# frankcholula/sapr

Hardware: AMD Instinct MI355X
Metric: frames/sec MFCC+Viterbi (16kHz, 13-MFCC, 8-state HMM) (higher is better)
Workload: dtype f32 (MFCC) + f64 (trellis); 1 GPU; configs[1]+[2]: 16 kHz 1 s utterances -> 13 MFCC (25 ms/10 ms, n_fft 512, 40 mels) -> Viterbi vs 11 word models x 8 emitting states (decoder.py API), features materialised in HBM; utterances_per_gpu=100000, frames_per_utterance=101, word_models=11, states=10, parallelism=utterance-shard x1, decoder=pruned

## Files before the change

### sapr_amd/csrc/mfcc.hip

```cpp
#include <cmath>
#include <algorithm>
#include <cstdlib>
#include <cstring>
#include <functional>
#include <mutex>
#include <type_traits>
#include <vector>

#include "sapr_common.h"

#pragma clang fp contract(fast)

#ifndef SAPR_ABLATE
#define SAPR_ABLATE 0
#endif

namespace sapr {
namespace {

constexpr int kThreads = 256;
constexpr int kWaves = kThreads / kWave;
constexpr double kPi = 3.14159265358979323846264338327950288;

typedef float f32x4 __attribute__((ext_vector_type(4)));
// ... 1213 lines not shown
    const char *sel = std::getenv("SAPR_MFCC_MEL");
    d.mel_bf16 = (d.ksr && sel && std::strcmp(sel, "bf16") == 0) ? 1 : 0;
  }
  auto lds_total = [&](int ml) {
    const int tp = d.two_pass ? 0 : d.t_pad;
    return R == 16 ? lds_layout<16>(tp, d.lm_stride, d.total_ks, ml, d.n_mels, d.stage_floats).total
                   : lds_layout<32>(tp, d.lm_stride, d.total_ks, ml, d.n_mels, d.stage_floats).total;
  };
  auto pick_mel = [&]() {
    if (d.ksr) return 0;
    return lds_total(1) <= 80 * 1024 || (lds_total(0) > 80 * 1024 && lds_total(1) <= 160 * 1024) ? 1 : 0;
  };
  d.mel_in_lds = pick_mel();
  if (!d.two_pass && lds_total(d.mel_in_lds) > 160 * 1024) {
    d.two_pass = 1;
    d.mel_in_lds = pick_mel();
  }
  if (!d.two_pass && lds_total(d.mel_in_lds) > 80 * 1024) {
    const char *keep = std::getenv("SAPR_MFCC_FUSED");
    MfccDev t = d;
    t.two_pass = 1;
    auto total_of = [&](const MfccDev &x, int ml) {
      return R == 16 ? lds_layout<16>(0, x.lm_stride, x.total_ks, ml, x.n_mels, x.stage_floats).total
                     : lds_layout<32>(0, x.lm_stride, x.total_ks, ml, x.n_mels, x.stage_floats).total;
    };
    const int ml2 = t.ksr ? 0 : ((total_of(t, 1) <= 80 * 1024 || (total_of(t, 0) > 80 * 1024 && total_of(t, 1) <= 160 * 1024)) ? 1 : 0);
    if (!(keep && keep[0] == '1') && total_of(t, ml2) <= 80 * 1024) {
      d.two_pass = 1;
      d.mel_in_lds = ml2;
    }
  }
  pl->lds_bytes = static_cast<size_t>(lds_total(d.mel_in_lds));
  if (pl->lds_bytes > 160 * 1024) {
    (void)hipFree(devbuf);
    const size_t need = pl->lds_bytes;
    delete pl;
    return fail(SAPR_ERR_UNSUPPORTED, "configuration needs %zu bytes of LDS (> 160 KiB)", need);
  }
  if (d.wave_s4) {
    d.two_pass = 1;
    pl->wave_rlo = (d.r_lo >= 1 && d.r_hi <= 15) ? 1 : 0;
    pl->wave_rhi = (d.r_lo >= 1 && d.r_hi <= 15) ? 15 : 16;
    pl->wave_lds = static_cast<size_t>(wave_lds(d.wave_s4, wave_region_floats(d.n_mels, d.deltas)).total);
    pl->lds_bytes = pl->wave_lds;
    hipError_t oe = wave_dispatch(*pl, &pl->wave_blocks_per_cu, nullptr, nullptr, nullptr, 0, 0, 1, nullptr, nullptr,
                                  nullptr, 0, nullptr);
    if (oe != hipSuccess || pl->wave_blocks_per_cu < 1) {
      (void)hipFree(devbuf);
      delete pl;
      return hip_fail(oe, "occupancy query (mfcc_wave_kernel)");
    }
    if (const char *sl = std::getenv("SAPR_MFCC_SLICES")) {
      const int v = std::atoi(sl);
      pl->slices_env = v < 1 ? 0 : (v > kMaxSlices ? kMaxSlices : v);
    }
    {
      int dev = 0, lds_cu = 0;
      if (hipGetDevice(&dev) != hipSuccess ||
          hipDeviceGetAttribute(&lds_cu, hipDeviceAttributeMaxSharedMemoryPerMultiprocessor, dev) != hipSuccess ||
          lds_cu < 64 * 1024)
        lds_cu = 160 * 1024;
      constexpr int kGranule = 320 * 4;
      const int spec = align_up(static_cast<int>(pl->wave_lds), kGranule) * pl->wave_blocks_per_cu;
      const int fin = align_up(static_cast<int>(wave_finish_lds(d.n_mels, d.deltas)), kGranule);
      const int fit = spec < lds_cu ? (lds_cu - spec) / fin : 0;
      pl->finish_beside = fit < 1 ? 1 : (fit > SAPR_FINISH_OCC ? SAPR_FINISH_OCC : fit);
    }
  }
  *plan_out = pl;
  return 0;
}

extern "C" int sapr_mfcc_plan_destroy(void *plan) {
  if (!plan) return 0;
  MfccPlan *pl = static_cast<MfccPlan *>(plan);
  plan_side_destroy(*pl, nullptr);
  if (pl->buffer) (void)hipFree(pl->buffer);
  delete pl;
  return 0;
}

extern "C" int sapr_mfcc_plan_info(const void *plan, int32_t *d_out, int32_t *max_frames,
                                   int64_t *lds_bytes, int32_t *mel_ksteps) {
  SAPR_REQUIRE(plan != nullptr, "plan is NULL");
  const MfccPlan *pl = static_cast<const MfccPlan *>(plan);
  if (d_out) *d_out = pl->dev.d_out;
  if (max_frames) *max_frames = pl->dev.two_pass ? 0 : pl->dev.t_pad;
  if (lds_bytes) *lds_bytes = static_cast<int64_t>(pl->lds_bytes);
  if (mel_ksteps) *mel_ksteps = pl->dev.total_ks;
  return 0;
}

extern "C" int sapr_mfcc_batch_stamped(const void *plan, const float *pcm, const int64_t *sample_offsets,
                                       const int64_t *frame_offsets, int64_t n_utts, float *out,
                                       int32_t grid_blocks, uint64_t *stamps, void *stream) {
  SAPR_REQUIRE(plan && pcm && sample_offsets && frame_offsets && out && stamps, "NULL pointer argument");
  const MfccPlan *pl = static_cast<const MfccPlan *>(plan);
  SAPR_REQUIRE(pl->R == 16 && pl->dev.preemph == 0.f && pl->dev.ksr == kKsr, "stamped build: bench preset only");
  SAPR_REQUIRE(grid_blocks > 0 && grid_blocks <= n_utts, "bad grid");
  if (pl->dev.mel_bf16) {
    if (pl->lds_bytes > 64 * 1024)
      SAPR_HIP_TRY(hipFuncSetAttribute(reinterpret_cast<const void *>(&mfcc_kernel<16, false, false, kKsr, true, false, true>),
                                       hipFuncAttributeMaxDynamicSharedMemorySize, static_cast<int>(pl->lds_bytes)));
    SAPR_LAUNCH((mfcc_kernel<16, false, false, kKsr, true, false, true>), dim3(grid_blocks), dim3(kThreads),
                pl->lds_bytes, as_stream(stream), pcm, sample_offsets, frame_offsets, n_utts, pl->dev, out,
                reinterpret_cast<unsigned long long *>(stamps));
  } else {
    if (pl->lds_bytes > 64 * 1024)
      SAPR_HIP_TRY(hipFuncSetAttribute(reinterpret_cast<const void *>(&mfcc_kernel<16, false, false, kKsr, true>),
                                       hipFuncAttributeMaxDynamicSharedMemorySize, static_cast<int>(pl->lds_bytes)));
    SAPR_LAUNCH((mfcc_kernel<16, false, false, kKsr, true>), dim3(grid_blocks), dim3(kThreads), pl->lds_bytes,
                as_stream(stream), pcm, sample_offsets, frame_offsets, n_utts, pl->dev, out,
                reinterpret_cast<unsigned long long *>(stamps));
  }
  SAPR_HIP_TRY(hipGetLastError());
  return 0;
}

extern "C" int sapr_mfcc_workspace_bytes(const void *plan, int64_t total_frames, int64_t n_utts, size_t *bytes) {
  SAPR_REQUIRE(plan && bytes && total_frames >= 0 && n_utts >= 0, "bad arguments");
  const MfccPlan *pl = static_cast<const MfccPlan *>(plan);
  *bytes = pl->dev.two_pass
               ? (static_cast<size_t>(total_frames) * pl->dev.n_mels + static_cast<size_t>(n_utts)) * sizeof(float) + 256
               : 0;
  return 0;
}

extern "C" int sapr_mfcc_batch(const void *plan, const float *pcm, const int64_t *sample_offsets,
                               const int64_t *frame_offsets, int64_t n_utts, int64_t total_frames, float *out,
                               int32_t grid_blocks, void *workspace, size_t workspace_size, void *stream) {
  SAPR_REQUIRE(plan != nullptr, "plan is NULL");
  SAPR_REQUIRE(n_utts >= 0 && total_frames >= 0, "bad sizes");
  if (n_utts == 0) return 0;
  SAPR_REQUIRE(pcm && sample_offsets && frame_offsets && out, "NULL pointer argument");
  const MfccPlan *pl = static_cast<const MfccPlan *>(plan);
  int dev = 0, cus = 256;
  SAPR_HIP_TRY(hipGetDevice(&dev));
  SAPR_HIP_TRY(hipDeviceGetAttribute(&cus, hipDeviceAttributeMultiprocessorCount, dev));
  int grid = grid_blocks;
  if (grid <= 0) {
    const int per_cu = static_cast<int>((160 * 1024) / pl->lds_bytes);
    const int cap = 3;
    grid = cus * (per_cu < 1 ? 1 : (per_cu > cap ? cap : per_cu));
  }
  if (grid > n_utts) grid = static_cast<int>(n_utts);
  hipStream_t st = as_stream(stream);
  if (!pl->dev.two_pass) {
    if (pl->R == 16)
      SAPR_HIP_TRY((launch<16, false>(*pl, pcm, sample_offsets, frame_offsets, n_utts, out, grid, st, nullptr, nullptr)));
    else
      SAPR_HIP_TRY((launch<32, false>(*pl, pcm, sample_offsets, frame_offsets, n_utts, out, grid, st, nullptr, nullptr)));
    return 0;
  }
  const size_t need = (static_cast<size_t>(total_frames) * pl->dev.n_mels + static_cast<size_t>(n_utts)) * sizeof(float) + 256;
  if (!workspace || workspace_size < need)
    return fail(SAPR_ERR_WORKSPACE, "two-pass MFCC plan needs a %zu-byte workspace (sapr_mfcc_workspace_bytes)", need);
  float *lm = static_cast<float *>(workspace);
  unsigned *gmax = reinterpret_cast<unsigned *>(lm + static_cast<size_t>(total_frames) * pl->dev.n_mels);
  if (pl->dev.wave_s4) {
    const int full_grid = cus * pl->wave_blocks_per_cu;
    const int64_t n_waves_full = static_cast<int64_t>(full_grid) * kWaves;
    const size_t flds = wave_finish_lds(pl->dev.n_mels, pl->dev.deltas);
    const int64_t *fo_end = frame_offsets + n_utts;
    auto finish = [&](hipStream_t s, int64_t u0, int64_t n, int fgrid, int fill) -> hipError_t {
      const int64_t fwaves = static_cast<int64_t>(fgrid) * kWaves;
      int fsplit = 1;
      if (n < fwaves) {
        fsplit = static_cast<int>(std::min<int64_t>(8, fwaves / n));
        const int64_t need_blocks = (n * fsplit + kWaves - 1) / kWaves;
        if (need_blocks < fgrid) fgrid = static_cast<int>(need_blocks);
      }
      SAPR_LAUNCH(mfcc_wave_finish_kernel, dim3(fgrid), dim3(kThreads), flds, s, lm, gmax + u0, frame_offsets + u0, n,
                  pl->dev, out, fsplit, total_frames, fo_end, fill);
      return hipGetLastError();
    };

    int n_slices = 1;
    if (grid_blocks <= 0 && pl->slices_env != 1) {
      if (pl->slices_env > 1) {
        n_slices = pl->slices_env;
      } else {
        n_slices = kDefaultSlices;
        const int64_t fwaves = static_cast<int64_t>(cus) * SAPR_FINISH_OCC * kWaves;
        while (n_slices > 1 && (n_utts / n_slices < fwaves || total_frames / n_slices < 4 * kSliceMinSets * n_waves_full))
          n_slices >>= 1;
      }
      if (n_slices > n_utts) n_slices = static_cast<int>(n_utts);
      if (n_slices > 1) {
        hipStreamCaptureStatus cap = hipStreamCaptureStatusNone;
        if (hipStreamIsCapturing(st, &cap) != hipSuccess || cap != hipStreamCaptureStatusNone) {
          (void)hipGetLastError();
          n_slices = 1;
        }
      }
    }
    if (n_slices > 1) {
      std::lock_guard<std::mutex> lock(pl->side_mu);
      if (!pl->side_tried) {
        pl->side_tried = true;
        int least = 0, greatest = 0;
        hipStream_t s = nullptr;
        bool ok = hipDeviceGetStreamPriorityRange(&least, &greatest) == hipSuccess &&
                  hipStreamCreateWithPriority(&s, hipStreamNonBlocking, least) == hipSuccess;
        for (int k = 0; ok && k < kMaxSlices; ++k) {
          hipEvent_t *e = k < kMaxSlices - 1 ? &pl->ev_spec[k] : &pl->ev_side;
          ok = hipEventCreateWithFlags(e, hipEventDisableTiming) == hipSuccess;
        }
        if (ok) {
          pl->side = s;
        } else {
          (void)hipGetLastError();
          plan_side_destroy(*pl, s);
        }
      }
      if (pl->side) {
        SAPR_HIP_TRY(hipMemsetAsync(gmax, 0, static_cast<size_t>(n_utts) * sizeof(unsigned), st));
        const int beside_grid = cus * pl->finish_beside;
        for (int k = 0; k < n_slices; ++k) {
          const int64_t u0 = n_utts * k / n_slices, n = n_utts * (k + 1) / n_slices - u0;
          SAPR_HIP_TRY(wave_dispatch(*pl, nullptr, pcm, sample_offsets + u0, frame_offsets + u0, n, full_grid, 0, st, lm,
                                     gmax + u0, total_frames, fo_end));
          if (k + 1 < n_slices) {
            SAPR_HIP_TRY(hipEventRecord(pl->ev_spec[k], st));
            SAPR_HIP_TRY(hipStreamWaitEvent(pl->side, pl->ev_spec[k], 0));
            SAPR_HIP_TRY(finish(pl->side, u0, n, beside_grid, 0));
          } else {
            SAPR_HIP_TRY(finish(st, u0, n, cus * SAPR_FINISH_OCC, 1));
          }
        }
        SAPR_HIP_TRY(hipEventRecord(pl->ev_side, pl->side));
        SAPR_HIP_TRY(hipStreamWaitEvent(st, pl->ev_side, 0));
        return 0;
      }
    }
    int wgrid = grid_blocks > 0 ? grid_blocks : full_grid;
    const int64_t n_waves = static_cast<int64_t>(wgrid) * kWaves;
    int64_t span = (total_frames + n_waves - 1) / n_waves;
    span = span < 4 ? 4 : (span + 3) / 4 * 4;
    const int64_t need_blocks = ((total_frames + span - 1) / span + kWaves - 1) / kWaves;
    if (need_blocks < wgrid) wgrid = static_cast<int>(need_blocks < 1 ? 1 : need_blocks);
    SAPR_HIP_TRY(hipMemsetAsync(gmax, 0, static_cast<size_t>(n_utts) * sizeof(unsigned), st));
    SAPR_HIP_TRY(wave_dispatch(*pl, nullptr, pcm, sample_offsets, frame_offsets, n_utts, wgrid, span, st, lm, gmax,
                               total_frames, fo_end));
    SAPR_HIP_TRY(finish(st, 0, n_utts, cus * SAPR_FINISH_OCC, 1));
    return 0;
  } else if (pl->R == 16)
    SAPR_HIP_TRY((launch<16, true>(*pl, pcm, sample_offsets, frame_offsets, n_utts, out, grid, st, lm, gmax)));
  else
    SAPR_HIP_TRY((launch<32, true>(*pl, pcm, sample_offsets, frame_offsets, n_utts, out, grid, st, lm, gmax)));
  int fgrid = cus * 6;
  if (fgrid > n_utts) fgrid = static_cast<int>(n_utts);
  SAPR_LAUNCH(mfcc_finish_kernel, dim3(fgrid), dim3(kThreads), finish_lds_bytes(pl->dev), st, lm, gmax, frame_offsets,
              n_utts, pl->dev, out);
  SAPR_HIP_TRY(hipGetLastError());
  return 0;
}
```

### sapr_amd/csrc/mfcc_wave.h

```cpp
#pragma once

constexpr int kWRowPad = 18;
constexpr int kWGroup = 16 * kWRowPad;
constexpr int kWRegion = 4 * kWGroup;
#include "mfcc_wave_pack.h"

struct WaveLds {
  int win, twab, twu, mela, dtab, scr, total;
};
__host__ __device__ inline int wave_region_floats(int, int) { return kWRegion; }
__host__ __device__ inline WaveLds wave_lds(int s4, int region_floats) {
  WaveLds L;
  int o = 0;
  L.win = o;
  o += 512 * 4;
  L.twab = o;
  o += 256 * 8;
  L.twu = o;
  o += 128 * 8;
  L.mela = o;
  o += s4 * kWave * 16;
  L.dtab = o;
  o += 2 * 81 * 4 + 8;
  L.scr = o;
// ... 161 lines not shown
#pragma unroll
        for (int c4 = 0; c4 < 4; ++c4) {
          const int idx = lane + kWave * c4;
          if (idx < rows * P.n_mfcc) {
            const int tl = static_cast<int>((static_cast<float>(idx) + 0.5f) * inv_nm), c = idx - tl * P.n_mfcc;
            const int t = 16 * e + tl;
            float d1 = 0.f, d2 = 0.f;
            if (t >= 4 && t < T - 4) {
#pragma unroll
              for (int k = 0; k < 9; ++k) {
                const float x = ceps(t - 4 + k, c);
                d1 += dc1[k] * x;
                d2 += dc2[k] * x;
              }
            } else {
              const int row = t < 4 ? 1 + t : 5 + (t - (T - 4)), t0 = t < 4 ? 0 : T - 9;
#pragma unroll
              for (int k = 0; k < 9; ++k) {
                const float x = ceps(t0 + k, c);
                d1 += s_dtab[row * 9 + k] * x;
                d2 += s_dtab[81 + row * 9 + k] * x;
              }
            }
            float *ot = o + tl * P.d_out + c;
            ot[0] = ceps(t, c);
            ot[P.n_mfcc] = d1;
            ot[2 * P.n_mfcc] = d2;
          }
        }
      }
      wave_fence();
    }
  };
  float4 t0[4], t1[4], t2[4];
  if (first < last) fetch(first, t0);
  if (first + 1 < last) fetch(first + 1, t1);
  if (first + 2 < last) fetch(first + 2, t2);
  const int end = last + (deltas ? 1 : 0);
  for (int base = first; base < end; base += 3) {
    tile(base, t0);
    if (base + 1 < end) tile(base + 1, t1);
    if (base + 2 < end) tile(base + 2, t2);
  }
}

#ifndef SAPR_FINISH_OCC
#define SAPR_FINISH_OCC 3
#endif
__global__ __launch_bounds__(kThreads, SAPR_FINISH_OCC) void mfcc_wave_finish_kernel(const float *__restrict__ lm,
                                                                       const unsigned *__restrict__ gmax_enc,
                                                                       const int64_t *__restrict__ frame_offsets,
                                                                       int64_t n_utts, MfccDev P, float *__restrict__ out,
                                                                       int split, int64_t total_cap,
                                                                       const int64_t *__restrict__ batch_end,
                                                                       int fill_on_mismatch) {
  extern __shared__ __attribute__((aligned(16))) unsigned char smem[];
  float *s_dtab = reinterpret_cast<float *>(smem);
  const int per_wave = 16 * (P.n_mels + 4) + (P.deltas ? 3 : 1) * 256;
  const int tid = threadIdx.x;
  const int wave = __builtin_amdgcn_readfirstlane(tid / kWave), lane = tid % kWave;
  for (int i = tid; i < 2 * 81; i += kThreads) s_dtab[i] = P.delta_tab[i];
  for (int i = tid; i < kWaves * per_wave; i += kThreads) s_dtab[168 + i] = 0.f;
  __syncthreads();
  float *s_tile = s_dtab + 168 + wave * per_wave;
  const int n_waves = gridDim.x * kWaves;
  const int wid = blockIdx.x * kWaves + wave;
  if (*batch_end > total_cap) {
    if (!fill_on_mismatch) return;
    const int64_t n = total_cap * P.d_out;
    for (int64_t i = static_cast<int64_t>(blockIdx.x) * kThreads + tid; i < n; i += static_cast<int64_t>(gridDim.x) * kThreads)
      out[i] = __builtin_nanf("");
    return;
  }
  const int n_teams = n_waves / split, part = wid % split;
  if (wid >= n_teams * split) return;
  for (int64_t u = wid / split; u < n_utts; u += n_teams) {
    const int64_t f_beg = frame_offsets[u];
    const int T = static_cast<int>(frame_offsets[u + 1] - f_beg);
    const int n_tiles = (T + 15) >> 4, per = (n_tiles + split - 1) / split;
    const int lo = part * per, hi = lo + per < n_tiles ? lo + per : n_tiles;
    if (lo >= hi) continue;
    wave_finish(lm + f_beg * P.n_mels, T, dec_ordered(gmax_enc[u]) - P.top_db, out + f_beg * P.d_out, P, s_tile,
                s_tile + 16 * (P.n_mels + 4), s_dtab, lane, lo, hi);
  }
}
inline size_t wave_finish_lds(int n_mels, int deltas) {
  return static_cast<size_t>(168 + kWaves * (16 * (n_mels + 4) + (deltas ? 3 : 1) * 256)) * 4;
}

#ifndef SAPR_WAVE_OCC
#define SAPR_WAVE_OCC 4
#endif

template <bool PREEMPH, int RLO, int RHI, int S4>
__global__ __launch_bounds__(kThreads, SAPR_WAVE_OCC) void mfcc_wave_kernel(
    const float *__restrict__ pcm, const int64_t *__restrict__ sample_offsets,
    const int64_t *__restrict__ frame_offsets, int64_t n_utts, MfccDev P, float *__restrict__ lm_out,
    unsigned *__restrict__ gmax_enc, int64_t span, int64_t total_cap, const int64_t *__restrict__ batch_end) {
  constexpr int R = 16, kNc = 256, kBits = 4, NR = RHI - RLO;
  extern __shared__ __attribute__((aligned(16))) unsigned char smem[];
  const int region_floats = wave_region_floats(P.n_mels, P.deltas);
  const WaveLds L = wave_lds(S4, region_floats);
  float *s_win = reinterpret_cast<float *>(smem + L.win);
  float2 *s_twab = reinterpret_cast<float2 *>(smem + L.twab);
  float2 *s_twu = reinterpret_cast<float2 *>(smem + L.twu);
  float4 *s_a = reinterpret_cast<float4 *>(smem + L.mela);
  float *s_dtab = reinterpret_cast<float *>(smem + L.dtab);
  float *s_scr = reinterpret_cast<float *>(smem + L.scr);

  const int tid = threadIdx.x;
  const int wave = __builtin_amdgcn_readfirstlane(tid / kWave);
  const int lane = tid % kWave;

  for (int i = tid; i < 512; i += kThreads) s_win[i] = P.window[i];
  for (int i = tid; i < 256; i += kThreads) s_twab[i] = P.tw_ab[i];
  for (int i = tid; i < 128; i += kThreads) s_twu[i] = P.tw_u[i];
  for (int i = tid; i < S4 * kWave; i += kThreads) s_a[i] = reinterpret_cast<const float4 *>(P.wave_a)[i];
  for (int i = tid; i < 2 * 81; i += kThreads) s_dtab[i] = P.delta_tab[i];
  for (int i = tid; i < kWaves * region_floats; i += kThreads) s_scr[i] = 0.f;
  __syncthreads();

  const int grp = lane >> 4;
  const int l = lane & 15;
  const int sigma = l < 8 ? l : (l == 15 ? 8 : l + 1);
  const bool is0 = l == 0;
  [[maybe_unused]] const bool special = l == 0 || l == 15;
  const unsigned long long special_mask = 0x8001800180018001ull;
  float *region = s_scr + wave * region_floats;
  float *scr = region + grp * kWGroup;
  float *prow = region + grp * kWPRow;
  const int rot = (grp & 1) * 8;
  float *wlo = scr + rot * kWRowPad + l;
  float *whi = scr + (rot ? -8 : 0) * kWRowPad + l;
  const unsigned a_rrow = lds_addr(scr + ((sigma + rot) & 15) * kWRowPad);
  const unsigned a_twu = lds_addr(s_twu + sigma);
  const unsigned a_twab = lds_addr(s_twab + l);
  const unsigned a_win = lds_addr(reinterpret_cast<const float2 *>(s_win) + l);

  const int j4 = lane & 3;
  const int4 bi = reinterpret_cast<const int4 *>(P.wave_blk)[lane >> 2];
  const float4 *bq = reinterpret_cast<const float4 *>(region + j4 * kWPRow + bi.x);
  const float4 *aq = s_a + lane;
  const int mel0 = bi.y;
  const float f1 = bi.z ? 1.f : 0.f, f2 = bi.w ? 1.f : 0.f;

  const int64_t base = frame_offsets[0], total = frame_offsets[n_utts];
  const int64_t wid = static_cast<int64_t>(blockIdx.x) * kWaves + wave;
  if (*batch_end > total_cap) return;
  if (span == 0) {
    const int64_t n_waves = static_cast<int64_t>(gridDim.x) * kWaves;
    span = (total - base + n_waves - 1) / n_waves;
    span = span < 4 ? 4 : (span + 3) / 4 * 4;
  }
  const int64_t run_lo = base + wid * span;
  if (run_lo >= total) return;
  const int64_t run_hi = run_lo + span < total ? run_lo + span : total;
  int64_t u_first = 0;
  {
    int64_t hi = n_utts;
    while (hi - u_first > 1) {
      const int64_t mid = (u_first + hi) >> 1;
      if (frame_offsets[mid] <= run_lo)
        u_first = mid;
      else
        hi = mid;
    }
  }

  for (int64_t u = u_first; u < n_utts; ++u) {
    const int64_t f_beg = frame_offsets[u];
    if (f_beg >= run_hi) break;
    const int T = static_cast<int>(frame_offsets[u + 1] - f_beg);
    const int n_sets = (T + 3) >> 2;
    const int s_lo = f_beg >= run_lo ? 0 : static_cast<int>((run_lo - f_beg + 3) >> 2);
    const int s_hi_raw = static_cast<int>((run_hi - f_beg + 3) >> 2);
    const int s_hi = s_hi_raw < n_sets ? s_hi_raw : n_sets;
    if (s_lo >= s_hi) continue;
    const int64_t s_beg = sample_offsets[u];
    const int n_samp = static_cast<int>(sample_offsets[u + 1] - s_beg);
    const __amdgpu_buffer_rsrc_t rsrc = __builtin_amdgcn_make_buffer_rsrc(
        const_cast<float *>(pcm + s_beg), 0, n_samp * 4, 0x00020000 );
    float run_max = -3.0e38f;

    WaveSet<PREEMPH, NR> nxt;
    auto issue = [&](int s) {
      const int vo = ((4 * s + grp) * P.hop - kNc + 2 * l) * 4;
      static_for<RLO, RHI>([&](auto r_c) {
        constexpr int r = decltype(r_c)::value;
        nxt.y[r - RLO] = __builtin_bit_cast(f2u, __builtin_amdgcn_raw_buffer_load_b64(rsrc, vo + 8 * R * r, 0, 0));
      });
      if constexpr (PREEMPH)
        nxt.m0 = __builtin_bit_cast(float, __builtin_amdgcn_raw_buffer_load_b32(rsrc, vo + 8 * R * RLO - 4, 0, 0));
    };
    issue(s_lo);

    for (int s = s_lo; s < s_hi; ++s) {
      float re[R], im[R];
      {
        v2f w[NR];
        static_for<RLO, RHI>([&](auto r_c) {
          constexpr int r = decltype(r_c)::value;
          w[r - RLO] = ds_rd64<8 * R * r>(a_win);
        });
        const int n0 = (4 * s + grp) * P.hop - kNc + 2 * l;
        const bool inside = (4 * s + 3) * P.hop + kNc <= n_samp;
        lds_wait();
        lds_dep(w);
        static_for<0, R>([&](auto r_c) {
          constexpr int r = decltype(r_c)::value;
          if constexpr (r < RLO || r >= RHI) {
            re[r] = 0.f;
            im[r] = 0.f;
          } else {
            f2u y = nxt.y[r - RLO];
            if constexpr (PREEMPH) {
              float m = nxt.m0;
              if constexpr (r > RLO) {
                const int wrap = __builtin_amdgcn_mov_dpp(__float_as_int(nxt.y[r - 1 - RLO].y), 0x121, 0xf, 0xf, true);
                m = __int_as_float(__builtin_amdgcn_update_dpp(wrap, __float_as_int(y.y), 0x111, 0xf, 0xf, false));
              }
              const float ya = y.x - P.preemph * m;
              const float yb = y.y - P.preemph * y.x;
              y.x = ya;
              y.y = yb;
              if (!inside) {
                const int idx = n0 + 2 * R * r;
                y.x = idx < n_samp ? y.x : 0.f;
                y.y = idx + 1 < n_samp ? y.y : 0.f;
              }
            }
            re[r] = y.x * w[r - RLO].x;
            im[r] = y.y * w[r - RLO].y;
          }
        });
      }
      {
        v2f tw[R - 1];
        static_for<1, R>([&](auto k1_c) {
          constexpr int k1 = decltype(k1_c)::value;
          tw[k1 - 1] = ds_rd64<8 * R * k1>(a_twab);
        });
        fft_inlane<R>(re, im);
        lds_wait();
        lds_dep(tw);
        static_for<1, R>([&](auto k1_c) {
          constexpr int k1 = decltype(k1_c)::value;
          constexpr int p = bitrev(k1, kBits);
          const float tr = re[p] * tw[k1 - 1].x - im[p] * tw[k1 - 1].y;
          const float ti = re[p] * tw[k1 - 1].y + im[p] * tw[k1 - 1].x;
          re[p] = tr;
          im[p] = ti;
        });
      }
      {
        v2f t[R / 2];
        static_for<0, R>([&](auto k1_c) {
          constexpr int k1 = decltype(k1_c)::value;
          (k1 < 8 ? wlo : whi)[k1 * kWRowPad] = re[bitrev(k1, kBits)];
        });
        static_for<0, R / 2>([&](auto c_c) {
          constexpr int c = decltype(c_c)::value;
          t[c] = ds_rd64_mem<8 * c>(a_rrow);
        });
        lds_wait();
        lds_dep(t);
        static_for<0, R / 2>([&](auto c_c) {
          constexpr int c = decltype(c_c)::value;
          re[2 * c] = t[c].x;
          re[2 * c + 1] = t[c].y;
        });
        static_for<0, R>([&](auto k1_c) {
          constexpr int k1 = decltype(k1_c)::value;
          (k1 < 8 ? wlo : whi)[k1 * kWRowPad] = im[bitrev(k1, kBits)];
        });
        static_for<0, R / 2>([&](auto c_c) {
          constexpr int c = decltype(c_c)::value;
          t[c] = ds_rd64_mem<8 * c>(a_rrow);
        });
        lds_wait();
        lds_dep(t);
        static_for<0, R / 2>([&](auto c_c) {
          constexpr int c = decltype(c_c)::value;
          im[2 * c] = t[c].x;
          im[2 * c + 1] = t[c].y;
        });
      }
      v2f tu[R / 2];
      static_for<0, R / 2>([&](auto k2_c) {
        constexpr int k2 = decltype(k2_c)::value;
        tu[k2] = ds_rd64<8 * R * k2>(a_twu);
      });
      fft_inlane<R>(re, im);
      lds_wait();
      lds_dep(tu);

      static_for<0, R / 2>([&](auto k2_c) {
        constexpr int k2 = decltype(k2_c)::value;
        constexpr int pz = bitrev(k2, kBits);
        constexpr int po = bitrev(R - 1 - k2, kBits);
        constexpr int ps = bitrev((R - k2) % R, kBits);
#if SAPR_WAVE_CNDDPP == 2
        float tr_, ti_;
        mirror_unless2_e64(re[po], im[po], special_mask, tr_, ti_);
        const float prr = is0 ? re[ps] : tr_, pii = is0 ? im[ps] : ti_;
#elif SAPR_WAVE_CNDDPP
        float tr_, ti_;
        mirror_unless2(re[po], im[po], special_mask, tr_, ti_);
        const float prr = is0 ? re[ps] : tr_, pii = is0 ? im[ps] : ti_;
#else
        const float selfr = is0 ? re[ps] : re[po], selfi = is0 ? im[ps] : im[po];
        const float mr = dpp_mov<0x140>(re[po]), mi = dpp_mov<0x140>(im[po]);
        const float prr = special ? selfr : mr, pii = special ? selfi : mi;
#endif
        const float zr = re[pz], zi = im[pz];
        const float er = zr + prr, ei = zi - pii;
        const float o_r = zi + pii, o_i = prr - zr;
        const float wx = tu[k2].x, wy = tu[k2].y;
        const float ar = __builtin_fmaf(wx, o_r, __builtin_fmaf(-wy, o_i, er));
        const float ai = __builtin_fmaf(wx, o_i, __builtin_fmaf(wy, o_r, ei));
        const float br = __builtin_fmaf(2.0f, er, -ar), bi2 = __builtin_fmaf(2.0f, ei, -ai);
        prow[sigma + R * k2] = ar * ar + ai * ai;
        prow[kNc - sigma - R * k2] = br * br + bi2 * bi2;
      });
      if (is0) {
        constexpr int pm = bitrev(R / 2, kBits);
        prow[kNc / 2] = 4.f * (re[pm] * re[pm] + im[pm] * im[pm]);
      }
      __builtin_amdgcn_fence(__ATOMIC_RELEASE, "wavefront");
      __builtin_amdgcn_wave_barrier();
      __builtin_amdgcn_fence(__ATOMIC_ACQUIRE, "wavefront");

      if (s + 1 < s_hi) issue(s + 1);

      f32x4 acc0 = {0.f, 0.f, 0.f, 0.f}, acc1 = {0.f, 0.f, 0.f, 0.f};
      {
        float4 a[S4], bv[S4];
#if SAPR_WAVE_FRAG64
        {
          const unsigned a_aq = lds_addr(aq), a_bq = lds_addr(bq);
          v2f t[4 * S4];
          static_for<0, S4>([&](auto q_c) {
            constexpr int q = decltype(q_c)::value;
            t[4 * q] = ds_rd64<q * kWave * 16>(a_aq);
            t[4 * q + 1] = ds_rd64<q * kWave * 16 + 8>(a_aq);
            t[4 * q + 2] = ds_rd64_mem<q * 16>(a_bq);
            t[4 * q + 3] = ds_rd64_mem<q * 16 + 8>(a_bq);
          });
          lds_wait();
          lds_dep(t);
#pragma unroll
          for (int q = 0; q < S4; ++q) {
            a[q] = float4{t[4 * q].x, t[4 * q].y, t[4 * q + 1].x, t[4 * q + 1].y};
            bv[q] = float4{t[4 * q + 2].x, t[4 * q + 2].y, t[4 * q + 3].x, t[4 * q + 3].y};
          }
        }
#else
#pragma unroll
        for (int q = 0; q < S4; ++q) {
          a[q] = aq[q * kWave];
          bv[q] = bq[q];
        }
#endif
#pragma unroll
        for (int q = 0; q < S4; ++q) {
          acc0 = __builtin_amdgcn_mfma_f32_4x4x1f32(a[q].x, bv[q].x, acc0, 0, 0, 0);
          acc1 = __builtin_amdgcn_mfma_f32_4x4x1f32(a[q].y, bv[q].y, acc1, 0, 0, 0);
          acc0 = __builtin_amdgcn_mfma_f32_4x4x1f32(a[q].z, bv[q].z, acc0, 0, 0, 0);
          acc1 = __builtin_amdgcn_mfma_f32_4x4x1f32(a[q].w, bv[q].w, acc1, 0, 0, 0);
        }
      }
      float e[4];
#pragma unroll
      for (int i = 0; i < 4; ++i) e[i] = acc0[i] + acc1[i];
#pragma unroll
      for (int i = 0; i < 4; ++i) e[i] += f1 * dpp_mov<0x104>(e[i]);
#pragma unroll
      for (int i = 0; i < 4; ++i) e[i] += f2 * dpp_mov<0x108>(e[i]);
      const int t = 4 * s + j4;
      if (mel0 >= 0 && t < T) {
        constexpr float kDb = 3.01029995663981195f;
        float4 v;
        v.x = kDb * __builtin_amdgcn_logf(fmaxf(P.amin, e[0]));
        v.y = kDb * __builtin_amdgcn_logf(fmaxf(P.amin, e[1]));
        v.z = kDb * __builtin_amdgcn_logf(fmaxf(P.amin, e[2]));
        v.w = kDb * __builtin_amdgcn_logf(fmaxf(P.amin, e[3]));
        int mel0_here = mel0;
        asm volatile("" : "+v"(mel0_here));
        *reinterpret_cast<float4 *>(lm_out + ((f_beg + t) * P.n_mels + mel0_here)) = v;
        run_max = fmaxf(run_max, fmaxf(fmaxf(v.x, v.y), fmaxf(v.z, v.w)));
      }
    }
#pragma unroll
    for (int o = 32; o > 0; o >>= 1) run_max = fmaxf(run_max, __shfl_xor(run_max, o, kWave));
    if (lane == 0) {
      if (s_lo == 0 && s_hi == n_sets)
        gmax_enc[u] = enc_ordered(run_max);
      else
        atomicMax(gmax_enc + u, enc_ordered(run_max));
    }
  }
}
```

Measured before the change: 2.055 billion frames/s.

## Pack frames across utterance boundaries in wave-per-span MFCC kernel

Reworks the wave-level MFCC loop to step over global frame sets of four instead of per-utterance sets, so a set of four frames can straddle utterance boundaries. This removes the partial-set padding at each utterance tail (101 frames leaves idle lanes in the last set) and replaces 64-bit offset arithmetic with 32-bit, wave-uniform readfirstlane values. It adds a rolling current/next utterance tracker with buffer-resource rebuilds, a slow path for boundary sets, and always uses atomicMax for per-utterance maxima. A host check now rejects batches near 2^31 frames or utterances.

```diff
diff --git a/sapr_amd/csrc/mfcc.hip b/sapr_amd/csrc/mfcc.hip
--- a/sapr_amd/csrc/mfcc.hip
+++ b/sapr_amd/csrc/mfcc.hip
@@ -1389,6 +1389,9 @@
       SAPR_HIP_TRY((launch<32, false>(*pl, pcm, sample_offsets, frame_offsets, n_utts, out, grid, st, nullptr, nullptr)));
     return 0;
   }
+  if (pl->dev.wave_s4)
+    SAPR_REQUIRE(total_frames < (int64_t{1} << 31) - 16 && n_utts < (int64_t{1} << 31) - 16,
+                 "2^31 - 16 frames or utterances or more in one batch");
   const size_t need = (static_cast<size_t>(total_frames) * pl->dev.n_mels + static_cast<size_t>(n_utts)) * sizeof(float) + 256;
   if (!workspace || workspace_size < need)
     return fail(SAPR_ERR_WORKSPACE, "two-pass MFCC plan needs a %zu-byte workspace (sapr_mfcc_workspace_bytes)", need);
diff --git a/sapr_amd/csrc/mfcc_wave.h b/sapr_amd/csrc/mfcc_wave.h
--- a/sapr_amd/csrc/mfcc_wave.h
+++ b/sapr_amd/csrc/mfcc_wave.h
@@ -337,251 +337,346 @@
     span = (total - base + n_waves - 1) / n_waves;
     span = span < 4 ? 4 : (span + 3) / 4 * 4;
   }
-  const int64_t run_lo = base + wid * span;
-  if (run_lo >= total) return;
-  const int64_t run_hi = run_lo + span < total ? run_lo + span : total;
-  int64_t u_first = 0;
+  if (wid * span >= total - base) return;
+  const int n_fr = static_cast<int>(total - base);
+  const int run_lo = static_cast<int>(wid * span);
+  const int run_hi = wid * span + span < n_fr ? run_lo + static_cast<int>(span) : n_fr;
+  const int n_u = static_cast<int>(n_utts);
+  auto fo_rel = [&](int u) {
+    return __builtin_amdgcn_readfirstlane(static_cast<int>(frame_offsets[u] - base));
+  };
+  auto so_at = [&](int u) {
+    const int64_t v = sample_offsets[u];
+    const unsigned lo = __builtin_amdgcn_readfirstlane(static_cast<int>(v));
+    const int hi = __builtin_amdgcn_readfirstlane(static_cast<int>(v >> 32));
+    return (static_cast<int64_t>(hi) << 32) | lo;
+  };
+  int u_first = 0;
   {
-    int64_t hi = n_utts;
+    int hi = n_u;
     while (hi - u_first > 1) {
-      const int64_t mid = (u_first + hi) >> 1;
-      if (frame_offsets[mid] <= run_lo)
+      const int mid = (u_first + hi) >> 1;
+      if (fo_rel(mid) <= run_lo)
         u_first = mid;
       else
         hi = mid;
     }
   }
-
-  for (int64_t u = u_first; u < n_utts; ++u) {
-    const int64_t f_beg = frame_offsets[u];
-    if (f_beg >= run_hi) break;
-    const int T = static_cast<int>(frame_offsets[u + 1] - f_beg);
-    const int n_sets = (T + 3) >> 2;
-    const int s_lo = f_beg >= run_lo ? 0 : static_cast<int>((run_lo - f_beg + 3) >> 2);
-    const int s_hi_raw = static_cast<int>((run_hi - f_beg + 3) >> 2);
-    const int s_hi = s_hi_raw < n_sets ? s_hi_raw : n_sets;
-    if (s_lo >= s_hi) continue;
-    const int64_t s_beg = sample_offsets[u];
-    const int n_samp = static_cast<int>(sample_offsets[u + 1] - s_beg);
-    const __amdgpu_buffer_rsrc_t rsrc = __builtin_amdgcn_make_buffer_rsrc(
-        const_cast<float *>(pcm + s_beg), 0, n_samp * 4, 0x00020000 );
-    float run_max = -3.0e38f;
-
-    WaveSet<PREEMPH, NR> nxt;
-    auto issue = [&](int s) {
-      const int vo = ((4 * s + grp) * P.hop - kNc + 2 * l) * 4;
+  auto utt_rsrc = [&](int64_t s_beg, int64_t s_end) {
+    return __builtin_amdgcn_make_buffer_rsrc(const_cast<float *>(pcm + s_beg), 0, static_cast<int>(s_end - s_beg) * 4,
+                                             0x00020000 );
+  };
+
+  int cu = u_first;
+  int cu_fb = fo_rel(cu), cu_fe = fo_rel(cu + 1);
+  int64_t cu_se = so_at(cu + 1);
+  __amdgpu_buffer_rsrc_t cu_rsrc = utt_rsrc(so_at(cu), cu_se);
+  int nx = cu + 1 < n_u ? cu + 1 : cu;
+  int nx_fe = fo_rel(nx + 1);
+  int64_t nx_se = so_at(nx + 1);
+  auto seek = [&](int f) {
+    while (cu_fe <= f && cu + 1 < n_u) {
+      cu = nx;
+      cu_fb = cu_fe;
+      cu_fe = nx_fe;
+      cu_rsrc = utt_rsrc(cu_se, nx_se);
+      cu_se = nx_se;
+      nx = cu + 1 < n_u ? cu + 1 : cu;
+      nx_fe = fo_rel(nx + 1);
+      nx_se = so_at(nx + 1);
+    }
+  };
+  auto for_each_utt = [&](int u0, int f0, auto fn) {
+    const int g_end = n_fr - f0 < 4 ? n_fr - f0 : 4;
+    int uu = u0;
+    for (int g = 0; g < g_end;) {
+      while (uu + 1 < n_u && fo_rel(uu + 1) <= f0 + g) ++uu;
+      const int fe = fo_rel(uu + 1);
+      const int g_hi = fe - f0 < g_end ? fe - f0 : g_end;
+      fn(g, g_hi, uu, fo_rel(uu), fe);
+      g = g_hi > g ? g_hi : g + 1;
+    }
+  };
+
+  WaveSet<PREEMPH, NR> nxt;
+  auto load_rows = [&](__amdgpu_buffer_rsrc_t rsrc, int t) {
+    const int vo = (t * P.hop - kNc + 2 * l) * 4;
+    static_for<RLO, RHI>([&](auto r_c) {
+      constexpr int r = decltype(r_c)::value;
+      nxt.y[r - RLO] = __builtin_bit_cast(f2u, __builtin_amdgcn_raw_buffer_load_b64(rsrc, vo + 8 * R * r, 0, 0));
+    });
+    if constexpr (PREEMPH)
+      nxt.m0 = __builtin_bit_cast(float, __builtin_amdgcn_raw_buffer_load_b32(rsrc, vo + 8 * R * RLO - 4, 0, 0));
+  };
+  auto issue = [&](int f0) {
+    seek(f0);
+    if (f0 + 4 <= cu_fe) {
+      load_rows(cu_rsrc, f0 - cu_fb + grp);
+    } else {
+#pragma unroll
+      for (int r = 0; r < NR; ++r) nxt.y[r] = f2u{0.f, 0.f};
+      if constexpr (PREEMPH) nxt.m0 = 0.f;
+      const int g_end = n_fr - f0 < 4 ? n_fr - f0 : 4;
+      for (int g = 0; g < g_end;) {
+        seek(f0 + g);
+        const int g_hi = cu_fe - f0 < g_end ? cu_fe - f0 : g_end;
+        if (grp >= g && grp < g_hi) load_rows(cu_rsrc, f0 - cu_fb + grp);
+        g = g_hi > g ? g_hi : g + 1;
+      }
+    }
+  };
+
+  seek(run_lo);
+  int u_run = cu;
+  int run_fb = cu_fb, run_fe = cu_fe;
+  [[maybe_unused]] int run_ns = PREEMPH ? static_cast<int>(cu_se - so_at(cu)) : 0;
+  float run_max = -3.0e38f;
+  auto flush_max = [&]() {
+#pragma unroll
+    for (int o = 32; o > 0; o >>= 1) run_max = fmaxf(run_max, __shfl_xor(run_max, o, kWave));
+    if (lane == 0) atomicMax(gmax_enc + u_run, enc_ordered(run_max));
+    run_max = -3.0e38f;
+  };
+  auto enter = [&](int uu, int fb, int fe) {
+    flush_max();
+    u_run = uu;
+    run_fb = fb;
+    run_fe = fe;
+    if constexpr (PREEMPH) run_ns = static_cast<int>(so_at(uu + 1) - so_at(uu));
+  };
+  float *set_rows = lm_out + (base + run_lo) * P.n_mels;
+  issue(run_lo);
+
+  for (int f0 = run_lo; f0 < run_hi; f0 += 4, set_rows += 4 * P.n_mels) {
+    auto next_utt = [&](int f) {
+      int uu = u_run + 1 < n_u ? u_run + 1 : u_run, fe = fo_rel(uu + 1);
+      while (fe <= f && uu + 1 < n_u) fe = fo_rel(++uu + 1);
+      enter(uu, run_fe, fe);
+    };
+    if (f0 >= run_fe) next_utt(f0);
+    const bool fast = f0 + 4 <= run_fe;
+    float re[R], im[R];
+    auto window = [&](int n0, bool inside, int ns) {
+      v2f w[NR];
       static_for<RLO, RHI>([&](auto r_c) {
         constexpr int r = decltype(r_c)::value;
-        nxt.y[r - RLO] = __builtin_bit_cast(f2u, __builtin_amdgcn_raw_buffer_load_b64(rsrc, vo + 8 * R * r, 0, 0));
-      });
-      if constexpr (PREEMPH)
-        nxt.m0 = __builtin_bit_cast(float, __builtin_amdgcn_raw_buffer_load_b32(rsrc, vo + 8 * R * RLO - 4, 0, 0));
+        w[r - RLO] = ds_rd64<8 * R * r>(a_win);
+      });
+      lds_wait();
+      lds_dep(w);
+      static_for<0, R>([&](auto r_c) {
+        constexpr int r = decltype(r_c)::value;
+        if constexpr (r < RLO || r >= RHI) {
+          re[r] = 0.f;
+          im[r] = 0.f;
+        } else {
+          f2u y = nxt.y[r - RLO];
+          if constexpr (PREEMPH) {
+            float m = nxt.m0;
+            if constexpr (r > RLO) {
+              const int wrap = __builtin_amdgcn_mov_dpp(__float_as_int(nxt.y[r - 1 - RLO].y), 0x121, 0xf, 0xf, true);
+              m = __int_as_float(__builtin_amdgcn_update_dpp(wrap, __float_as_int(y.y), 0x111, 0xf, 0xf, false));
+            }
+            const float ya = y.x - P.preemph * m;
+            const float yb = y.y - P.preemph * y.x;
+            y.x = ya;
+            y.y = yb;
+            if (!inside) {
+              const int idx = n0 + 2 * R * r;
+              y.x = idx < ns ? y.x : 0.f;
+              y.y = idx + 1 < ns ? y.y : 0.f;
+            }
+          }
+          re[r] = y.x * w[r - RLO].x;
+          im[r] = y.y * w[r - RLO].y;
+        }
+      });
     };
-    issue(s_lo);
-
-    for (int s = s_lo; s < s_hi; ++s) {
-      float re[R], im[R];
+    if constexpr (!PREEMPH) {
+      window(0, true, 0);
+    } else if (fast) {
+      const int t0 = f0 - run_fb;
+      window((t0 + grp) * P.hop - kNc + 2 * l, (t0 + 3) * P.hop + kNc <= run_ns, run_ns);
+    } else {
+      int t_l = 0, ns_l = 0;
+      for_each_utt(u_run, f0, [&](int g_lo, int g_hi, int uu, int fb, int) {
+        const int ns = static_cast<int>(so_at(uu + 1) - so_at(uu));
+        if (grp >= g_lo && grp < g_hi) {
+          t_l = f0 - fb + grp;
+          ns_l = ns;
+        }
+      });
+      window(t_l * P.hop - kNc + 2 * l, false, ns_l);
+    }
+    {
+      v2f tw[R - 1];
+      static_for<1, R>([&](auto k1_c) {
+        constexpr int k1 = decltype(k1_c)::value;
+        tw[k1 - 1] = ds_rd64<8 * R * k1>(a_twab);
+      });
+      fft_inlane<R>(re, im);
+      lds_wait();
+      lds_dep(tw);
+      static_for<1, R>([&](auto k1_c) {
+        constexpr int k1 = decltype(k1_c)::value;
+        constexpr int p = bitrev(k1, kBits);
+        const float tr = re[p] * tw[k1 - 1].x - im[p] * tw[k1 - 1].y;
+        const float ti = re[p] * tw[k1 - 1].y + im[p] * tw[k1 - 1].x;
+        re[p] = tr;
+        im[p] = ti;
+      });
+    }
+    {
+      v2f t[R / 2];
+      static_for<0, R>([&](auto k1_c) {
+        constexpr int k1 = decltype(k1_c)::value;
+        (k1 < 8 ? wlo : whi)[k1 * kWRowPad] = re[bitrev(k1, kBits)];
+      });
+      static_for<0, R / 2>([&](auto c_c) {
+        constexpr int c = decltype(c_c)::value;
+        t[c] = ds_rd64_mem<8 * c>(a_rrow);
+      });
+      lds_wait();
+      lds_dep(t);
+      static_for<0, R / 2>([&](auto c_c) {
+        constexpr int c = decltype(c_c)::value;
+        re[2 * c] = t[c].x;
+        re[2 * c + 1] = t[c].y;
+      });
+      static_for<0, R>([&](auto k1_c) {
+        constexpr int k1 = decltype(k1_c)::value;
+        (k1 < 8 ? wlo : whi)[k1 * kWRowPad] = im[bitrev(k1, kBits)];
+      });
+      static_for<0, R / 2>([&](auto c_c) {
+        constexpr int c = decltype(c_c)::value;
+        t[c] = ds_rd64_mem<8 * c>(a_rrow);
+      });
+      lds_wait();
+      lds_dep(t);
+      static_for<0, R / 2>([&](auto c_c) {
+        constexpr int c = decltype(c_c)::value;
+        im[2 * c] = t[c].x;
+        im[2 * c + 1] = t[c].y;
+      });
+    }
+    v2f tu[R / 2];
+    static_for<0, R / 2>([&](auto k2_c) {
+      constexpr int k2 = decltype(k2_c)::value;
+      tu[k2] = ds_rd64<8 * R * k2>(a_twu);
+    });
+    fft_inlane<R>(re, im);
+    lds_wait();
+    lds_dep(tu);
+
+    static_for<0, R / 2>([&](auto k2_c) {
+      constexpr int k2 = decltype(k2_c)::value;
+      constexpr int pz = bitrev(k2, kBits);
+      constexpr int po = bitrev(R - 1 - k2, kBits);
+      constexpr int ps = bitrev((R - k2) % R, kBits);
+#if SAPR_WAVE_CNDDPP == 2
+      float tr_, ti_;
+      mirror_unless2_e64(re[po], im[po], special_mask, tr_, ti_);
+      const float prr = is0 ? re[ps] : tr_, pii = is0 ? im[ps] : ti_;
+#elif SAPR_WAVE_CNDDPP
+      float tr_, ti_;
+      mirror_unless2(re[po], im[po], special_mask, tr_, ti_);
+      const float prr = is0 ? re[ps] : tr_, pii = is0 ? im[ps] : ti_;
+#else
+      const float selfr = is0 ? re[ps] : re[po], selfi = is0 ? im[ps] : im[po];
+      const float mr = dpp_mov<0x140>(re[po]), mi = dpp_mov<0x140>(im[po]);
+      const float prr = special ? selfr : mr, pii = special ? selfi : mi;
+#endif
+      const float zr = re[pz], zi = im[pz];
+      const float er = zr + prr, ei = zi - pii;
+      const float o_r = zi + pii, o_i = prr - zr;
+      const float wx = tu[k2].x, wy = tu[k2].y;
+      const float ar = __builtin_fmaf(wx, o_r, __builtin_fmaf(-wy, o_i, er));
+      const float ai = __builtin_fmaf(wx, o_i, __builtin_fmaf(wy, o_r, ei));
+      const float br = __builtin_fmaf(2.0f, er, -ar), bi2 = __builtin_fmaf(2.0f, ei, -ai);
+      prow[sigma + R * k2] = ar * ar + ai * ai;
+      prow[kNc - sigma - R * k2] = br * br + bi2 * bi2;
+    });
+    if (is0) {
+      constexpr int pm = bitrev(R / 2, kBits);
+      prow[kNc / 2] = 4.f * (re[pm] * re[pm] + im[pm] * im[pm]);
+    }
+    __builtin_amdgcn_fence(__ATOMIC_RELEASE, "wavefront");
+    __builtin_amdgcn_wave_barrier();
+    __builtin_amdgcn_fence(__ATOMIC_ACQUIRE, "wavefront");
+
+    if (f0 + 4 < run_hi) issue(f0 + 4);
+
+    f32x4 acc0 = {0.f, 0.f, 0.f, 0.f}, acc1 = {0.f, 0.f, 0.f, 0.f};
+    {
+      float4 a[S4], bv[S4];
+#if SAPR_WAVE_FRAG64
       {
-        v2f w[NR];
-        static_for<RLO, RHI>([&](auto r_c) {
-          constexpr int r = decltype(r_c)::value;
-          w[r - RLO] = ds_rd64<8 * R * r>(a_win);
-        });
-        const int n0 = (4 * s + grp) * P.hop - kNc + 2 * l;
-        const bool inside = (4 * s + 3) * P.hop + kNc <= n_samp;
-        lds_wait();
-        lds_dep(w);
-        static_for<0, R>([&](auto r_c) {
-          constexpr int r = decltype(r_c)::value;
-          if constexpr (r < RLO || r >= RHI) {
-            re[r] = 0.f;
-            im[r] = 0.f;
-          } else {
-            f2u y = nxt.y[r - RLO];
-            if constexpr (PREEMPH) {
-              float m = nxt.m0;
-              if constexpr (r > RLO) {
-                const int wrap = __builtin_amdgcn_mov_dpp(__float_as_int(nxt.y[r - 1 - RLO].y), 0x121, 0xf, 0xf, true);
-                m = __int_as_float(__builtin_amdgcn_update_dpp(wrap, __float_as_int(y.y), 0x111, 0xf, 0xf, false));
-              }
-              const float ya = y.x - P.preemph * m;
-              const float yb = y.y - P.preemph * y.x;
-              y.x = ya;
-              y.y = yb;
-              if (!inside) {
-                const int idx = n0 + 2 * R * r;
-                y.x = idx < n_samp ? y.x : 0.f;
-                y.y = idx + 1 < n_samp ? y.y : 0.f;
-              }
-            }
-            re[r] = y.x * w[r - RLO].x;
-            im[r] = y.y * w[r - RLO].y;
-          }
-        });
-      }
-      {
-        v2f tw[R - 1];
-        static_for<1, R>([&](auto k1_c) {
-          constexpr int k1 = decltype(k1_c)::value;
-          tw[k1 - 1] = ds_rd64<8 * R * k1>(a_twab);
-        });
-        fft_inlane<R>(re, im);
-        lds_wait();
-        lds_dep(tw);
-        static_for<1, R>([&](auto k1_c) {
-          constexpr int k1 = decltype(k1_c)::value;
-          constexpr int p = bitrev(k1, kBits);
-          const float tr = re[p] * tw[k1 - 1].x - im[p] * tw[k1 - 1].y;
-          const float ti = re[p] * tw[k1 - 1].y + im[p] * tw[k1 - 1].x;
-          re[p] = tr;
-          im[p] = ti;
-        });
-      }
-      {
-        v2f t[R / 2];
-        static_for<0, R>([&](auto k1_c) {
-          constexpr int k1 = decltype(k1_c)::value;
-          (k1 < 8 ? wlo : whi)[k1 * kWRowPad] = re[bitrev(k1, kBits)];
-        });
-        static_for<0, R / 2>([&](auto c_c) {
-          constexpr int c = decltype(c_c)::value;
-          t[c] = ds_rd64_mem<8 * c>(a_rrow);
+        const unsigned a_aq = lds_addr(aq), a_bq = lds_addr(bq);
+        v2f t[4 * S4];
+        static_for<0, S4>([&](auto q_c) {
+          constexpr int q = decltype(q_c)::value;
+          t[4 * q] = ds_rd64<q * kWave * 16>(a_aq);
+          t[4 * q + 1] = ds_rd64<q * kWave * 16 + 8>(a_aq);
+          t[4 * q + 2] = ds_rd64_mem<q * 16>(a_bq);
+          t[4 * q + 3] = ds_rd64_mem<q * 16 + 8>(a_bq);
         });
         lds_wait();
         lds_dep(t);
-        static_for<0, R / 2>([&](auto c_c) {
-          constexpr int c = decltype(c_c)::value;
-          re[2 * c] = t[c].x;
-          re[2 * c + 1] = t[c].y;
-        });
-        static_for<0, R>([&](auto k1_c) {
-          constexpr int k1 = decltype(k1_c)::value;
-          (k1 < 8 ? wlo : whi)[k1 * kWRowPad] = im[bitrev(k1, kBits)];
-        });
-        static_for<0, R / 2>([&](auto c_c) {
-          constexpr int c = decltype(c_c)::value;
-          t[c] = ds_rd64_mem<8 * c>(a_rrow);
-        });
-        lds_wait();
-        lds_dep(t);
-        static_for<0, R / 2>([&](auto c_c) {
-          constexpr int c = decltype(c_c)::value;
-          im[2 * c] = t[c].x;
-          im[2 * c + 1] = t[c].y;
-        });
-      }
-      v2f tu[R / 2];
-      static_for<0, R / 2>([&](auto k2_c) {
-        constexpr int k2 = decltype(k2_c)::value;
-        tu[k2] = ds_rd64<8 * R * k2>(a_twu);
-      });
-      fft_inlane<R>(re, im);
-      lds_wait();
-      lds_dep(tu);
-
-      static_for<0, R / 2>([&](auto k2_c) {
-        constexpr int k2 = decltype(k2_c)::value;
-        constexpr int pz = bitrev(k2, kBits);
-        constexpr int po = bitrev(R - 1 - k2, kBits);
-        constexpr int ps = bitrev((R - k2) % R, kBits);
-#if SAPR_WAVE_CNDDPP == 2
-        float tr_, ti_;
-        mirror_unless2_e64(re[po], im[po], special_mask, tr_, ti_);
-        const float prr = is0 ? re[ps] : tr_, pii = is0 ? im[ps] : ti_;
-#elif SAPR_WAVE_CNDDPP
-        float tr_, ti_;
-        mirror_unless2(re[po], im[po], special_mask, tr_, ti_);
-        const float prr = is0 ? re[ps] : tr_, pii = is0 ? im[ps] : ti_;
+#pragma unroll
+        for (int q = 0; q < S4; ++q) {
+          a[q] = float4{t[4 * q].x, t[4 * q].y, t[4 * q + 1].x, t[4 * q + 1].y};
+          bv[q] = float4{t[4 * q + 2].x, t[4 * q + 2].y, t[4 * q + 3].x, t[4 * q + 3].y};
+        }
+      }
 #else
-        const float selfr = is0 ? re[ps] : re[po], selfi = is0 ? im[ps] : im[po];
-        const float mr = dpp_mov<0x140>(re[po]), mi = dpp_mov<0x140>(im[po]);
-        const float prr = special ? selfr : mr, pii = special ? selfi : mi;
+#pragma unroll
+      for (int q = 0; q < S4; ++q) {
+        a[q] = aq[q * kWave];
+        bv[q] = bq[q];
+      }
 #endif
-        const float zr = re[pz], zi = im[pz];
-        const float er = zr + prr, ei = zi - pii;
-        const float o_r = zi + pii, o_i = prr - zr;
-        const float wx = tu[k2].x, wy = tu[k2].y;
-        const float ar = __builtin_fmaf(wx, o_r, __builtin_fmaf(-wy, o_i, er));
-        const float ai = __builtin_fmaf(wx, o_i, __builtin_fmaf(wy, o_r, ei));
-        const float br = __builtin_fmaf(2.0f, er, -ar), bi2 = __builtin_fmaf(2.0f, ei, -ai);
-        prow[sigma + R * k2] = ar * ar + ai * ai;
-        prow[kNc - sigma - R * k2] = br * br + bi2 * bi2;
-      });
-      if (is0) {
-        constexpr int pm = bitrev(R / 2, kBits);
-        prow[kNc / 2] = 4.f * (re[pm] * re[pm] + im[pm] * im[pm]);
-      }
-      __builtin_amdgcn_fence(__ATOMIC_RELEASE, "wavefront");
-      __builtin_amdgcn_wave_barrier();
-      __builtin_amdgcn_fence(__ATOMIC_ACQUIRE, "wavefront");
-
-      if (s + 1 < s_hi) issue(s + 1);
-
-      f32x4 acc0 = {0.f, 0.f, 0.f, 0.f}, acc1 = {0.f, 0.f, 0.f, 0.f};
-      {
-        float4 a[S4], bv[S4];
-#if SAPR_WAVE_FRAG64
-        {
-          const unsigned a_aq = lds_addr(aq), a_bq = lds_addr(bq);
-          v2f t[4 * S4];
-          static_for<0, S4>([&](auto q_c) {
-            constexpr int q = decltype(q_c)::value;
-            t[4 * q] = ds_rd64<q * kWave * 16>(a_aq);
-            t[4 * q + 1] = ds_rd64<q * kWave * 16 + 8>(a_aq);
-            t[4 * q + 2] = ds_rd64_mem<q * 16>(a_bq);
-            t[4 * q + 3] = ds_rd64_mem<q * 16 + 8>(a_bq);
-          });
-          lds_wait();
-          lds_dep(t);
-#pragma unroll
-          for (int q = 0; q < S4; ++q) {
-            a[q] = float4{t[4 * q].x, t[4 * q].y, t[4 * q + 1].x, t[4 * q + 1].y};
-            bv[q] = float4{t[4 * q + 2].x, t[4 * q + 2].y, t[4 * q + 3].x, t[4 * q + 3].y};
-          }
-        }
-#else
-#pragma unroll
-        for (int q = 0; q < S4; ++q) {
-          a[q] = aq[q * kWave];
-          bv[q] = bq[q];
-        }
-#endif
-#pragma unroll
-        for (int q = 0; q < S4; ++q) {
-          acc0 = __builtin_amdgcn_mfma_f32_4x4x1f32(a[q].x, bv[q].x, acc0, 0, 0, 0);
-          acc1 = __builtin_amdgcn_mfma_f32_4x4x1f32(a[q].y, bv[q].y, acc1, 0, 0, 0);
-          acc0 = __builtin_amdgcn_mfma_f32_4x4x1f32(a[q].z, bv[q].z, acc0, 0, 0, 0);
-          acc1 = __builtin_amdgcn_mfma_f32_4x4x1f32(a[q].w, bv[q].w, acc1, 0, 0, 0);
-        }
-      }
-      float e[4];
-#pragma unroll
-      for (int i = 0; i < 4; ++i) e[i] = acc0[i] + acc1[i];
-#pragma unroll
-      for (int i = 0; i < 4; ++i) e[i] += f1 * dpp_mov<0x104>(e[i]);
-#pragma unroll
-      for (int i = 0; i < 4; ++i) e[i] += f2 * dpp_mov<0x108>(e[i]);
-      const int t = 4 * s + j4;
-      if (mel0 >= 0 && t < T) {
-        constexpr float kDb = 3.01029995663981195f;
-        float4 v;
-        v.x = kDb * __builtin_amdgcn_logf(fmaxf(P.amin, e[0]));
-        v.y = kDb * __builtin_amdgcn_logf(fmaxf(P.amin, e[1]));
-        v.z = kDb * __builtin_amdgcn_logf(fmaxf(P.amin, e[2]));
-        v.w = kDb * __builtin_amdgcn_logf(fmaxf(P.amin, e[3]));
-        int mel0_here = mel0;
-        asm volatile("" : "+v"(mel0_here));
-        *reinterpret_cast<float4 *>(lm_out + ((f_beg + t) * P.n_mels + mel0_here)) = v;
-        run_max = fmaxf(run_max, fmaxf(fmaxf(v.x, v.y), fmaxf(v.z, v.w)));
-      }
-    }
-#pragma unroll
-    for (int o = 32; o > 0; o >>= 1) run_max = fmaxf(run_max, __shfl_xor(run_max, o, kWave));
-    if (lane == 0) {
-      if (s_lo == 0 && s_hi == n_sets)
-        gmax_enc[u] = enc_ordered(run_max);
-      else
-        atomicMax(gmax_enc + u, enc_ordered(run_max));
-    }
-  }
-}
+#pragma unroll
+      for (int q = 0; q < S4; ++q) {
+        acc0 = __builtin_amdgcn_mfma_f32_4x4x1f32(a[q].x, bv[q].x, acc0, 0, 0, 0);
+        acc1 = __builtin_amdgcn_mfma_f32_4x4x1f32(a[q].y, bv[q].y, acc1, 0, 0, 0);
+        acc0 = __builtin_amdgcn_mfma_f32_4x4x1f32(a[q].z, bv[q].z, acc0, 0, 0, 0);
+        acc1 = __builtin_amdgcn_mfma_f32_4x4x1f32(a[q].w, bv[q].w, acc1, 0, 0, 0);
+      }
+    }
+    float e[4];
+#pragma unroll
+    for (int i = 0; i < 4; ++i) e[i] = acc0[i] + acc1[i];
+#pragma unroll
+    for (int i = 0; i < 4; ++i) e[i] += f1 * dpp_mov<0x104>(e[i]);
+#pragma unroll
+    for (int i = 0; i < 4; ++i) e[i] += f2 * dpp_mov<0x108>(e[i]);
+    auto store_row = [&]() {
+      constexpr float kDb = 3.01029995663981195f;
+      float4 v;
+      v.x = kDb * __builtin_amdgcn_logf(fmaxf(P.amin, e[0]));
+      v.y = kDb * __builtin_amdgcn_logf(fmaxf(P.amin, e[1]));
+      v.z = kDb * __builtin_amdgcn_logf(fmaxf(P.amin, e[2]));
+      v.w = kDb * __builtin_amdgcn_logf(fmaxf(P.amin, e[3]));
+      int mel0_here = mel0;
+      asm volatile("" : "+v"(mel0_here));
+      const unsigned lane_off = static_cast<unsigned>(j4 * P.n_mels + mel0_here) * 4u;
+      *reinterpret_cast<float4 *>(reinterpret_cast<char *>(set_rows) + lane_off) = v;
+      return fmaxf(fmaxf(v.x, v.y), fmaxf(v.z, v.w));
+    };
+    if (fast) {
+      if (mel0 >= 0) run_max = fmaxf(run_max, store_row());
+    } else {
+      float vm = -3.0e38f;
+      if (mel0 >= 0 && f0 + j4 < n_fr) vm = store_row();
+      const int g_end = n_fr - f0 < 4 ? n_fr - f0 : 4;
+      for (int g = 0;;) {
+        const int g_hi = run_fe - f0 < g_end ? run_fe - f0 : g_end;
+        run_max = fmaxf(run_max, j4 >= g && j4 < g_hi ? vm : -3.0e38f);
+        g = g_hi > g ? g_hi : g + 1;
+        if (g >= g_end) break;
+        next_utt(f0 + g);
+      }
+    }
+  }
+  flush_max();
+}
```

New measurement: 2.116 billion frames/s (median of 6 runs). 2.9% higher.
